# OpenDriveLab/Vista

Measured on NVIDIA H100. Metric: denoised frames/sec at 25x576x1024, 50 EDM steps; UNet step ms, higher is better.
Workload: dtype f16 (fp32 accumulate, fp32 norms/softmax/sampler state)

## Files before the change

vista_b200/csrc/gemm_tc.cu:

```cuda
#include "gemm_tc.cuh"

namespace vb {
extern template const GemmKern* gemm_variants<32>();
extern template const GemmKern* gemm_variants<64>();
extern template const GemmKern* gemm_variants<96>();
extern template const GemmKern* gemm_variants<128>();
extern template const GemmKern* gemm_variants<160>();
extern template const GemmKern* gemm_variants<192>();
extern template const GemmKern* gemm_variants<224>();
extern template const GemmKern* gemm_variants<256>();
}

extern "C" int b200v_gemm(const b200v_gemm_desc* d, void* stream_) {
  using namespace vb;
  cudaStream_t stream = reinterpret_cast<cudaStream_t>(stream_);
  VB_REQUIRE(d && d->a && d->b && d->out, "b200v_gemm: null pointer");
  VB_REQUIRE(d->cin > 0 && d->cin % 64 == 0, "b200v_gemm: cin=%d must be a positive multiple of 64", d->cin);
  VB_REQUIRE(d->ntaps >= 1 && d->ntaps <= 9, "b200v_gemm: ntaps=%d out of range", d->ntaps);
  VB_REQUIRE(d->N > 0 && d->N % 8 == 0, "b200v_gemm: N=%d must be a multiple of 8", d->N);
  VB_REQUIRE(d->tile_n >= 32 && d->tile_n <= 256 && d->tile_n % 32 == 0, "b200v_gemm: tile_n=%d invalid", d->tile_n);
  VB_REQUIRE(d->lda % 8 == 0 && d->ldo % 8 == 0, "b200v_gemm: lda/ldo must be multiples of 8");
  VB_REQUIRE(d->act >= 0 && d->act <= 3, "b200v_gemm: act=%d invalid", d->act);
  VB_REQUIRE(!(d->act == 2 && (d->tile_n % 64 != 0 || d->N % d->tile_n != 0 || d->out_f32)),
             "b200v_gemm: GEGLU needs tile_n %% 64 == 0, N %% tile_n == 0, 16-bit output");
  VB_REQUIRE(!(d->act == 2 && (d->rowvec || d->res1 || d->res2)), "b200v_gemm: GEGLU epilogue takes bias only");
  VB_REQUIRE(!(d->act == 3 && (d->rowvec || d->res1 || d->res2 || d->bf16 || d->out_f32 || d->stats)),
             "b200v_gemm: the GELU epilogue takes bias only, fp16 operands and output (compiled variant)");
  VB_REQUIRE(!d->res1 || d->ld_res1 % 8 == 0, "b200v_gemm: ld_res1 must be a multiple of 8");
  VB_REQUIRE(!d->res2 || d->ld_res2 % 8 == 0, "b200v_gemm: ld_res2 must be a multiple of 8");
  VB_REQUIRE(!d->rowvec || (d->ld_rowvec % 4 == 0 && d->rv_div > 0 && d->rv_mod > 0), "b200v_gemm: bad rowvec args");
  VB_REQUIRE((reinterpret_cast<uintptr_t>(d->a) & 15) == 0 && (reinterpret_cast<uintptr_t>(d->b) & 15) == 0 &&
                 (reinterpret_cast<uintptr_t>(d->out) & 15) == 0,
             "b200v_gemm: a/b/out must be 16-byte aligned");

  TGParams p;
  memset(&p, 0, sizeof(p));
  p.a_mode = d->a_mode;
  p.tokens = d->tokens;
  const long long K = (long long)d->ntaps * d->cin;
  CUtensorMap tmA, tmB;
  if (d->a_mode == 0) {
    VB_REQUIRE(d->ntaps == 1 && d->h_pad == 0, "b200v_gemm: linear mode takes one tap and no halo rows");
    VB_REQUIRE(d->tokens > 0 && d->tokens < (1ll << 31) - 256, "b200v_gemm: tokens out of range");
    p.W = (int)d->tokens; p.H = 1; p.NB = 1;
    p.BW = 128; p.BH = 1; p.BB = 1;
    p.tiles_w = (int)((d->tokens + 127) / 128); p.tiles_h = 1;
    p.m_tiles = p.tiles_w;
    uint64_t dims[2] = {(uint64_t)d->cin, (uint64_t)d->tokens};
    uint64_t strides[1] = {(uint64_t)d->lda * 2};
    uint32_t box[2] = {64, 128};
    uint32_t es[2] = {1, 1};
    if (encode_tmap_16bit(&tmA, d->a, 2, dims, strides, box, es, d->bf16)) return 3;
  } else {
    VB_REQUIRE(d->a_mode == 1 || d->a_mode == 2, "b200v_gemm: a_mode=%d invalid", d->a_mode);
    const long long out_tokens = d->a_mode == 2 ? 4ll * d->tokens : d->tokens;
    VB_REQUIRE(d->W > 0 && d->H > 0 && d->NB > 0 && (long long)d->W * d->H * d->NB == d->tokens &&
                   out_tokens < (1ll << 31) - 256,
               "b200v_gemm: W*H*NB != tokens (or output tokens >= 2^31)");
    VB_REQUIRE(d->a_mode == 1 || (d->h_pad == 0 && d->act == 0 && !d->rowvec && !d->res1 && !d->res2 && !d->bf16 &&
                                  !d->out_f32 && d->s_acc == 1.0f),
               "b200v_gemm: the upsampling mode (a_mode 2) takes bias and fused statistics only, fp16 in and out");
    VB_REQUIRE(d->box_w > 0 && d->box_h > 0 && d->box_b > 0 && d->box_w * d->box_h * d->box_b == 128,
               "b200v_gemm: box_w*box_h*box_b must be 128");
    p.W = d->W; p.H = d->H; p.NB = d->NB;
    p.BW = d->box_w; p.BH = d->box_h; p.BB = d->box_b;
    p.tiles_w = (d->W + p.BW - 1) / p.BW;
    p.tiles_h = (d->H + p.BH - 1) / p.BH;
    const int tiles_b = (d->NB + p.BB - 1) / p.BB;
    p.m_tiles = p.tiles_w * p.tiles_h * tiles_b * (d->a_mode == 2 ? 4 : 1);
    VB_REQUIRE(d->h_pad >= 0 && d->h_pad <= 4, "b200v_gemm: h_pad=%d out of range", d->h_pad);
    const uint64_t He = (uint64_t)d->H + 2ull * d->h_pad;
    uint64_t dims[4] = {(uint64_t)d->cin, (uint64_t)d->W, He, (uint64_t)d->NB};
    uint64_t strides[3] = {(uint64_t)d->lda * 2, (uint64_t)d->lda * 2 * d->W, (uint64_t)d->lda * 2 * d->W * He};
    uint32_t box[4] = {64, (uint32_t)p.BW, (uint32_t)p.BH, (uint32_t)p.BB};
    uint32_t es[4] = {1, 1, 1, 1};
    if (encode_tmap_16bit(&tmA, d->a, 4, dims, strides, box, es, d->bf16)) return 3;
  }
  {
    uint64_t dims[2] = {(uint64_t)K, (uint64_t)d->N};
    uint64_t strides[1] = {(uint64_t)K * 2};
    uint32_t box[2] = {64, (uint32_t)d->tile_n};
    uint32_t es[2] = {1, 1};
    if (encode_tmap_16bit(&tmB, d->b, 2, dims, strides, box, es, d->bf16)) return 3;
  }
  p.ntaps = d->ntaps;
  p.kc_per_tap = d->cin / 64;
  for (int i = 0; i < 9; ++i) {
    p.dh[i] = d->dh[i] + (d->a_mode == 1 ? d->h_pad : 0);
    p.dw[i] = d->dw[i];
  }
  p.N = d->N;
  p.n_tiles = (d->N + d->tile_n - 1) / d->tile_n;
  p.stage_bytes = kABytes + ((d->tile_n * 128 + 1023) / 1024) * 1024;
  constexpr int kMaxSmem = 227 * 1024;
  p.nstages = (kMaxSmem - 2048 - kStagingBytes) / p.stage_bytes;
  if (p.nstages > kMaxStages) p.nstages = kMaxStages;
  const long long kMaxLd = (1ll << 31) - 1;
  VB_REQUIRE(d->ldo * (d->out_f32 ? 4 : 2) <= kMaxLd && d->ld_rowvec * 4 <= kMaxLd && d->ld_res1 * 2 <= kMaxLd &&
                 d->ld_res2 * 2 <= kMaxLd,
             "b200v_gemm: row stride too large");
  for (p.bw_sh = 0; (1 << p.bw_sh) < p.BW; ++p.bw_sh) {}
  for (p.bh_sh = 0; (1 << p.bh_sh) < p.BH; ++p.bh_sh) {}
  p.out = d->out; p.ldo_b = (int)(d->ldo * (d->out_f32 ? 4 : 2)); p.out_f32 = d->out_f32; p.act = d->act;
  p.bias = d->bias;
  p.rowvec = d->rowvec; p.ld_rowvec_b = (int)(d->ld_rowvec * 4); p.rv_div = d->rv_div > 0 ? d->rv_div : 1;
  p.rv_mod = d->rv_mod > 0 ? d->rv_mod : 1;
  p.res1 = d->res1; p.ld_res1_b = (int)(d->ld_res1 * 2); p.s_res1 = d->s_res1;
  p.res2 = d->res2; p.ld_res2_b = (int)(d->ld_res2 * 2); p.s_res2 = d->s_res2;
  p.s_acc = d->s_acc;
  VB_REQUIRE(!(d->res2 && !d->res1), "b200v_gemm: res2 without res1");
  p.stats = d->stats; p.stats_ld = (int)d->stats_ld; p.stats_col0 = d->stats_col0;
  if (d->stats) {
    VB_REQUIRE(!d->bf16 && !d->out_f32 && d->act == 0 && !d->res2 && !(d->rowvec && d->res1),
               "b200v_gemm: fused statistics need fp16 output, act 0, <= 1 residual and no rowvec + residual");
    VB_REQUIRE(d->stats_ld >= d->stats_col0 + d->N && d->stats_col0 % 4 == 0 && d->stats_ld % 4 == 0 &&
                   (reinterpret_cast<uintptr_t>(d->stats) & 15) == 0,
               "b200v_gemm: bad stats_ld / stats_col0 / alignment");
    VB_REQUIRE(d->a_mode == 0 || (p.BB == 1 && d->W % p.BW == 0 && d->H % p.BH == 0 &&
                                  (d->a_mode == 2 || p.BW == d->W || p.BH == 1)),
               "b200v_gemm: fused statistics need token tiles of 128 consecutive tokens, or boxes that tile each frame "
               "in upsampling mode (box %d x %d x %d on %d x %d)",
               p.BW, p.BH, p.BB, d->W, d->H);
  }

  const int smem_bytes = 1024 + 1024 + p.nstages * p.stage_bytes + kStagingBytes;
  int variant = d->bf16 ? 12 : 7;
  if (d->stats) {
    variant = 9 + (d->rowvec ? 2 : (d->res1 ? 1 : 0));
  } else if (!d->bf16 && !d->out_f32) {
    const int nres = (d->res1 ? 1 : 0) + (d->res2 ? 1 : 0);
    if (d->act == 0 && !d->rowvec) variant = nres;
    else if (d->act == 0 && nres <= 1) variant = 3 + nres;
    else if (d->act == 1 && !d->rowvec && nres == 0) variant = 5;
    else if (d->act == 2) variant = 6;
    else if (d->act == 3) variant = 8;
  }
  static const GemmKern* const kByWidth[8] = {gemm_variants<32>(),  gemm_variants<64>(),  gemm_variants<96>(),
                                              gemm_variants<128>(), gemm_variants<160>(), gemm_variants<192>(),
                                              gemm_variants<224>(), gemm_variants<256>()};
  static bool attr_set[64] = {false};
  if (vb::first_use_on_device(attr_set)) {
    for (int w = 0; w < 8; ++w)
      for (int i = 0; i < kGemmVariants; ++i)
        VB_CHECK_CUDA(cudaFuncSetAttribute(kByWidth[w][i], cudaFuncAttributeMaxDynamicSharedMemorySize, kMaxSmem));
  }
  const long long total = (long long)p.m_tiles * p.n_tiles;
  int grid = device_sm_count();
  if (total < grid) grid = (int)total;
  const GemmKern k = kByWidth[d->tile_n / 32 - 1][variant];
  k<<<grid, kGemmThreads, smem_bytes, stream>>>(tmA, tmB, p);
  VB_CHECK_CUDA(cudaGetLastError());
  return 0;
}
```

vista_b200/csrc/gemm_tc.cuh:

```cuda
#pragma once
#include "../../include/vista_b200.h"
#include "host.cuh"
#include "ptx.cuh"

namespace vb {

constexpr int kMaxStages = 8;
constexpr int kABytes = 128 * 64 * 2;
constexpr int kStageBufBytes = 64 * 32 * 4;
constexpr int kStagingBytes = 2 * 2 * kStageBufBytes;
constexpr int kGemmThreads = 384;

struct TGParams {
  int a_mode;
  int W, H, NB;
  int BW, BH, BB;
  int bw_sh, bh_sh;
  int tiles_w, tiles_h;
  int m_tiles, n_tiles;
  int ntaps, kc_per_tap;
  int dh[9], dw[9];
  int N;
  int nstages, stage_bytes;
  long long tokens;
  void* out;
  int ldo_b;
  int out_f32, act;
  const float* bias;
  const float* rowvec;
  int ld_rowvec_b;
  int rv_div, rv_mod;
  const void* res1;
  int ld_res1_b;
  float s_res1;
  const void* res2;
  int ld_res2_b;
  float s_res2;
  float s_acc;
  float* stats;
  int stats_ld, stats_col0;
};

__device__ __forceinline__ float2 unpack2(uint32_t w, int bf16) {
  if (bf16) return make_float2(__uint_as_float(w << 16), __uint_as_float(w & 0xFFFF0000u));
  return __half22float2(*reinterpret_cast<const __half2*>(&w));
}
__device__ __forceinline__ uint32_t pack2(float a, float b, int bf16) {
  if (bf16) {
    __nv_bfloat162 t = __floats2bfloat162_rn(a, b);
    return *reinterpret_cast<uint32_t*>(&t);
  }
  __half2 t = __floats2half2_rn(a, b);
  return *reinterpret_cast<uint32_t*>(&t);
}

template <int TN, bool BF16>
__device__ __forceinline__ void issue_kchunk(float (&acc)[TN / 2], uint64_t adesc, uint64_t bdesc, bool overwrite) {
#pragma unroll
  for (int kk = 0; kk < 4; ++kk)
    wgmma_ss<TN, BF16>(acc, adesc + (uint64_t)(2 * kk), bdesc + (uint64_t)(2 * kk), (overwrite && kk == 0) ? 0 : 1);
}

template <int TN, int ACT_, bool RV_, int NRES_, bool GEN, bool STATS = false, bool BF16 = false>
__global__ void __launch_bounds__(kGemmThreads, 1)
tapgemm_kernel(const __grid_constant__ CUtensorMap tmA, const __grid_constant__ CUtensorMap tmB, const TGParams p) {
  extern __shared__ uint8_t smem_raw[];
  const uint32_t raw = smem_u32(smem_raw);
  uint8_t* smem = smem_raw + (((raw + 1023u) & ~1023u) - raw);
  uint64_t* full = reinterpret_cast<uint64_t*>(smem);
  uint64_t* empty = full + kMaxStages;
  uint8_t* stages = smem + 1024;

  const int warp = threadIdx.x >> 5, lane = threadIdx.x & 31;
  const int KC = p.ntaps * p.kc_per_tap;
  const int total_tiles = p.m_tiles * p.n_tiles;

  if (threadIdx.x == 0) {
    for (int i = 0; i < p.nstages; ++i) {
      mbar_init(&full[i], 1);
      mbar_init(&empty[i], 8);
    }
    fence_barrier_init();
  }
  if (warp == 8 && lane == 0) {
    tma_prefetch_desc(&tmA);
    tma_prefetch_desc(&tmB);
  }
  __syncthreads();

  if (warp >= 8) {
    setmaxnreg_dec<40>();
    if (warp == 8 && lane == 0) {
      int stage = 0;
      uint32_t phase = 0;
      const uint32_t tx = (uint32_t)(kABytes + TN * 128);
      for (int tile = blockIdx.x; tile < total_tiles; tile += gridDim.x) {
        const int m_blk = tile / p.n_tiles, n_blk = tile - m_blk * p.n_tiles;
        const int up = p.a_mode == 2;
        const int box = up ? (m_blk >> 2) : m_blk;
        const int px = up ? (m_blk & 1) : 0, py = up ? ((m_blk >> 1) & 1) : 0;
        const int tw = box % p.tiles_w;
        const int th = (box / p.tiles_w) % p.tiles_h;
        const int tb = box / (p.tiles_w * p.tiles_h);
        const int w0 = tw * p.BW, h0 = th * p.BH, b0 = tb * p.BB;
        const int n0 = n_blk * TN;
        for (int kc = 0; kc < KC; ++kc) {
          mbar_wait_relaxed(&empty[stage], phase ^ 1, 1);
          uint8_t* sA = stages + stage * p.stage_bytes;
          uint8_t* sB = sA + kABytes;
          const int tap = kc / p.kc_per_tap;
          const int c0 = (kc - tap * p.kc_per_tap) * 64;
          mbar_expect_tx(&full[stage], tx);
          const int dw = up ? ((px + p.dw[tap]) >> 1) : p.dw[tap];
          const int dh = up ? ((py + p.dh[tap]) >> 1) : p.dh[tap];
          if (p.a_mode == 0)
            tma_load_2d(sA, &tmA, &full[stage], c0, w0);
          else
            tma_load_4d(sA, &tmA, &full[stage], c0, w0 + dw, h0 + dh, b0);
          tma_load_2d(sB, &tmB, &full[stage], kc * 64, n0);
          if (++stage == p.nstages) {
            stage = 0;
            phase ^= 1;
          }
        }
      }
    }
    return;
  }

  setmaxnreg_inc<232>();
  const int wg = warp >> 2, wq = warp & 3;
  const int act = GEN ? p.act : ACT_;
  const bool has_rv = GEN ? (p.rowvec != nullptr) : RV_;
  const bool has_r1 = GEN ? (p.res1 != nullptr) : (NRES_ >= 1);
  const bool has_r2 = GEN ? (p.res2 != nullptr) : (NRES_ >= 2);
  constexpr bool bf16 = BF16;
  const bool f32o = GEN ? (p.out_f32 != 0) : false;
  const bool has_bias = p.bias != nullptr;
  constexpr int half = TN >> 1;
  const int tile_out_cols = (act == 2) ? half : TN;
  const int n_out_total = (act == 2) ? (p.N >> 1) : p.N;
  const int G = tile_out_cols >> 5;
  const int out_es = f32o ? 4 : 2;
  const char* r1p = reinterpret_cast<const char*>(p.res1);
  const char* r2p = reinterpret_cast<const char*>(p.res2);
  const uint64_t desc0 = make_desc_sw128(smem_u32(stages), 16, 1024);
  const uint32_t stage_step = (uint32_t)p.stage_bytes >> 4;
  const uint32_t stg0 = smem_u32(stages + p.nstages * p.stage_bytes) + wg * 2 * kStageBufBytes;
  const int g = lane >> 2, c = lane & 3;
  const int rh = wq & 1, chh = wq >> 1;
  const int ch = lane & 3, rsub = lane >> 2;
  int stage = 0;
  uint32_t phase = 0;
  uint32_t gcount = 0;

  float acc[TN / 2];
  for (int tile = blockIdx.x; tile < total_tiles; tile += gridDim.x) {
    const int m_blk = tile / p.n_tiles, n_blk = tile - m_blk * p.n_tiles;
    int prev = -1;
    for (int kc = 0; kc < KC; ++kc) {
      mbar_wait(&full[stage], phase, 3);
      const uint64_t ad = desc0 + (uint64_t)(stage * stage_step + wg * 512);
      const uint64_t bd = desc0 + (uint64_t)(stage * stage_step + (kABytes >> 4));
      wgmma_fence();
      issue_kchunk<TN, BF16>(acc, ad, bd, kc == 0);
      wgmma_commit();
      if (prev >= 0) {
        wgmma_wait<1>();
        if (lane == 0) mbar_arrive(&empty[prev]);
      }
      prev = stage;
      if (++stage == p.nstages) {
        stage = 0;
        phase ^= 1;
      }
    }
    wgmma_wait<0>();
    if (lane == 0) mbar_arrive(&empty[prev]);
    fence_regs(acc);

    const int r_own = wg * 64 + rh * 32 + lane;
    int token_own, valid_own;
    if (p.a_mode == 0) {
      token_own = m_blk * 128 + r_own;
      valid_own = token_own < p.tokens;
    } else {
      const int up = p.a_mode == 2;
      const int box = up ? (m_blk >> 2) : m_blk;
      const int tw = box % p.tiles_w;
      const int t2 = box / p.tiles_w;
      const int th = t2 % p.tiles_h;
      const int tb = t2 / p.tiles_h;
      const int ww = r_own & (p.BW - 1), hh = (r_own >> p.bw_sh) & (p.BH - 1), bb = r_own >> (p.bw_sh + p.bh_sh);
      const int w = tw * p.BW + ww, h = th * p.BH + hh, b = tb * p.BB + bb;
      valid_own = (w < p.W) && (h < p.H) && (b < p.NB);
      token_own = up ? ((2 * (b * p.H + h) + ((m_blk >> 1) & 1)) * 2 * p.W + 2 * w + (m_blk & 1))
                     : (b * p.H + h) * p.W + w;
    }
    if (!valid_own) token_own = 0;
    const uint32_t vrows = __ballot_sync(0xffffffffu, valid_own) >> rsub;
    int tok[4], rvrow[4];
    {
      const int rv_own = has_rv ? (token_own / p.rv_div) % p.rv_mod : 0;
#pragma unroll
      for (int i = 0; i < 4; ++i) {
        tok[i] = __shfl_sync(0xffffffffu, token_own, i * 8 + rsub);
        rvrow[i] = has_rv ? __shfl_sync(0xffffffffu, rv_own, i * 8 + rsub) : 0;
      }
    }
    const int n_out_base = n_blk * tile_out_cols;
#pragma unroll
    for (int k = 0; k < TN / 32; ++k) {
      if (k >= G) break;
      const int c0 = k * 32;
      if (n_out_base + c0 >= n_out_total) break;
      const uint32_t stg = stg0 + (gcount & 1) * kStageBufBytes;
      ++gcount;
      float f[16];
#pragma unroll
      for (int j = 0; j < 16; ++j) f[j] = acc[16 * k + j];
      if (act == 2) {
        float gt[16];
        const int kg = (half >> 5) + k;
#pragma unroll
        for (int j = 0; j < 16; ++j) gt[j] = 0.f;
#pragma unroll
        for (int q = 0; q < TN / 32; ++q)
          if (q == kg) {
#pragma unroll
            for (int j = 0; j < 16; ++j) gt[j] = acc[16 * q + j];
          }
        const int nb = n_blk * TN + c0;
#pragma unroll
        for (int ii = 0; ii < 4; ++ii) {
          float2 bv = make_float2(0.f, 0.f), bg = make_float2(0.f, 0.f);
          if (has_bias) {
            bv = __ldg(reinterpret_cast<const float2*>(p.bias + nb + 8 * ii + 2 * c));
            bg = __ldg(reinterpret_cast<const float2*>(p.bias + nb + half + 8 * ii + 2 * c));
          }
          f[4 * ii + 0] = geglu_fast(f[4 * ii + 0] + bv.x, gt[4 * ii + 0] + bg.x);
          f[4 * ii + 1] = geglu_fast(f[4 * ii + 1] + bv.y, gt[4 * ii + 1] + bg.y);
          f[4 * ii + 2] = geglu_fast(f[4 * ii + 2] + bv.x, gt[4 * ii + 2] + bg.x);
          f[4 * ii + 3] = geglu_fast(f[4 * ii + 3] + bv.y, gt[4 * ii + 3] + bg.y);
        }
      }
#pragma unroll
      for (int ii = 0; ii < 4; ++ii) {
        const int chunk = 2 * ii + (c >> 1), sub = (c & 1) * 8;
#pragma unroll
        for (int hr = 0; hr < 2; ++hr) {
          const int row = wq * 16 + g + 8 * hr;
          asm volatile("st.shared.v2.f32 [%0], {%1, %2};" ::"r"(stg + row * 128 + ((chunk ^ (row & 7)) << 4) + sub),
                       "f"(f[4 * ii + 2 * hr]), "f"(f[4 * ii + 2 * hr + 1])
                       : "memory");
        }
      }
      asm volatile("bar.sync %0, 128;" ::"r"(1 + wg) : "memory");
      {
        const int n = n_out_base + c0 + chh * 16 + ch * 4;
        const bool n_ok = n + 4 <= n_out_total;
        float4 bs = make_float4(0.f, 0.f, 0.f, 0.f);
        float sa = 1.0f;
        if (act != 2) {
          sa = p.s_acc;
          if (has_bias && n_ok) {
            const float4 b4 = __ldg(reinterpret_cast<const float4*>(p.bias + n));
            bs = make_float4(b4.x * sa, b4.y * sa, b4.z * sa, b4.w * sa);
          }
        }
        char* obase = reinterpret_cast<char*>(p.out) + (long long)n * out_es;
        const char* r1base = r1p + (long long)n * 2;
        const char* r2base = r2p + (long long)n * 2;
        const char* rvbase = reinterpret_cast<const char*>(p.rowvec) + (long long)n * 4;
        float cs[4] = {0.f, 0.f, 0.f, 0.f}, cq[4] = {0.f, 0.f, 0.f, 0.f};
        float4 v[4], rv[4];
        uint2 u1[4], u2[4];
#pragma unroll
        for (int i = 0; i < 4; ++i) {
          const int row = rh * 32 + i * 8 + rsub;
          const int chunk = chh * 4 + ch;
          asm volatile("ld.shared.v4.f32 {%0, %1, %2, %3}, [%4];"
                       : "=f"(v[i].x), "=f"(v[i].y), "=f"(v[i].z), "=f"(v[i].w)
                       : "r"(stg + row * 128 + ((chunk ^ (row & 7)) << 4)));
          const bool ok = n_ok && ((vrows >> (8 * i)) & 1u);
          rv[i] = make_float4(0.f, 0.f, 0.f, 0.f);
          u1[i] = make_uint2(0, 0);
          u2[i] = make_uint2(0, 0);
          if (has_rv && ok) rv[i] = __ldg(reinterpret_cast<const float4*>(rvbase + (long long)rvrow[i] * p.ld_rowvec_b));
          if (has_r1 && ok) u1[i] = __ldg(reinterpret_cast<const uint2*>(r1base + (long long)tok[i] * p.ld_res1_b));
          if (has_r2 && ok) u2[i] = __ldg(reinterpret_cast<const uint2*>(r2base + (long long)tok[i] * p.ld_res2_b));
        }
#pragma unroll
        for (int i = 0; i < 4; ++i) {
          const bool ok = n_ok && ((vrows >> (8 * i)) & 1u);
          float4 o = v[i];
          if (act != 2) {
            o.x = fmaf(o.x, sa, bs.x); o.y = fmaf(o.y, sa, bs.y); o.z = fmaf(o.z, sa, bs.z); o.w = fmaf(o.w, sa, bs.w);
            if (has_rv) { o.x += rv[i].x; o.y += rv[i].y; o.z += rv[i].z; o.w += rv[i].w; }
            if (act == 1) { o.x = silu_f(o.x); o.y = silu_f(o.y); o.z = silu_f(o.z); o.w = silu_f(o.w); }
            if (!GEN && act == 3) { o.x = gelu_erf_fast(o.x); o.y = gelu_erf_fast(o.y); o.z = gelu_erf_fast(o.z); o.w = gelu_erf_fast(o.w); }
            if (has_r1) {
              const float2 a = unpack2(u1[i].x, bf16), b = unpack2(u1[i].y, bf16);
              o.x = fmaf(p.s_res1, a.x, o.x); o.y = fmaf(p.s_res1, a.y, o.y);
              o.z = fmaf(p.s_res1, b.x, o.z); o.w = fmaf(p.s_res1, b.y, o.w);
            }
            if (has_r2) {
              const float2 a = unpack2(u2[i].x, bf16), b = unpack2(u2[i].y, bf16);
              o.x = fmaf(p.s_res2, a.x, o.x); o.y = fmaf(p.s_res2, a.y, o.y);
              o.z = fmaf(p.s_res2, b.x, o.z); o.w = fmaf(p.s_res2, b.y, o.w);
            }
          }
          if (STATS && ok) {
            cs[0] += o.x; cs[1] += o.y; cs[2] += o.z; cs[3] += o.w;
            cq[0] = fmaf(o.x, o.x, cq[0]); cq[1] = fmaf(o.y, o.y, cq[1]);
            cq[2] = fmaf(o.z, o.z, cq[2]); cq[3] = fmaf(o.w, o.w, cq[3]);
          }
          char* optr = obase + (long long)tok[i] * p.ldo_b;
          if (f32o) {
            if (ok) *reinterpret_cast<float4*>(optr) = o;
          } else {
            const uint2 pk = make_uint2(pack2(o.x, o.y, bf16), pack2(o.z, o.w, bf16));
            if (ok) *reinterpret_cast<uint2*>(optr) = pk;
          }
        }
        if (STATS) {
#pragma unroll
          for (int off = 4; off < 32; off <<= 1) {
#pragma unroll
            for (int q = 0; q < 4; ++q) {
              cs[q] += __shfl_xor_sync(0xffffffffu, cs[q], off);
              cq[q] += __shfl_xor_sync(0xffffffffu, cq[q], off);
            }
          }
          if (rsub == 0 && n_ok) {
            float* dst = p.stats + (((long long)m_blk * 4 + wg * 2 + rh) * p.stats_ld + p.stats_col0 + n) * 2;
            *reinterpret_cast<float4*>(dst) = make_float4(cs[0], cq[0], cs[1], cq[1]);
            *reinterpret_cast<float4*>(dst + 4) = make_float4(cs[2], cq[2], cs[3], cq[3]);
          }
        }
      }
    }
  }
}

using GemmKern = void (*)(const CUtensorMap, const CUtensorMap, const TGParams);
constexpr int kGemmVariants = 13;

template <int TN>
const GemmKern* gemm_variants() {
  static const GemmKern v[kGemmVariants] = {
      tapgemm_kernel<TN, 0, false, 0, false>,       tapgemm_kernel<TN, 0, false, 1, false>,
      tapgemm_kernel<TN, 0, false, 2, false>,       tapgemm_kernel<TN, 0, true, 0, false>,
      tapgemm_kernel<TN, 0, true, 1, false>,        tapgemm_kernel<TN, 1, false, 0, false>,
      tapgemm_kernel<TN, 2, false, 0, false>,       tapgemm_kernel<TN, 0, true, 2, true>,
      tapgemm_kernel<TN, 3, false, 0, false>,       tapgemm_kernel<TN, 0, false, 0, false, true>,
      tapgemm_kernel<TN, 0, false, 1, false, true>, tapgemm_kernel<TN, 0, true, 0, false, true>,
      tapgemm_kernel<TN, 0, true, 2, true, false, true>};
  return v;
}

}
```

vista_b200/csrc/host.cu:

```cuda
#include <stdarg.h>

#include <mutex>

#include "../../include/vista_b200.h"
#include "host.cuh"

namespace vb {

static thread_local char g_err[1024] = "";

void set_error(const char* fmt, ...) {
  va_list ap;
  va_start(ap, fmt);
  vsnprintf(g_err, sizeof(g_err), fmt, ap);
  va_end(ap);
}
const char* last_error() { return g_err; }

int device_sm_count() {
  static int cached[64] = {0};
  int dev = 0;
  if (cudaGetDevice(&dev) != cudaSuccess || dev < 0 || dev >= 64) return 132;
  if (cached[dev] == 0) {
    int n = 0;
    if (cudaDeviceGetAttribute(&n, cudaDevAttrMultiProcessorCount, dev) != cudaSuccess || n <= 0) n = 132;
    cached[dev] = n;
  }
  return cached[dev];
}

typedef CUresult (*EncodeTiledFn)(CUtensorMap*, CUtensorMapDataType, cuuint32_t, void*, const cuuint64_t*,
                                  const cuuint64_t*, const cuuint32_t*, const cuuint32_t*, CUtensorMapInterleave,
                                  CUtensorMapSwizzle, CUtensorMapL2promotion, CUtensorMapFloatOOBfill);

static EncodeTiledFn get_encode_fn() {
  static EncodeTiledFn fn = nullptr;
  static std::once_flag once;
  std::call_once(once, [] {
    void* p = nullptr;
    cudaDriverEntryPointQueryResult q;
    if (cudaGetDriverEntryPoint("cuTensorMapEncodeTiled", &p, cudaEnableDefault, &q) == cudaSuccess &&
        q == cudaDriverEntryPointSuccess)
      fn = reinterpret_cast<EncodeTiledFn>(p);
  });
  return fn;
}

int encode_tmap_16bit(CUtensorMap* out, const void* base, int rank, const uint64_t* dims,
                      const uint64_t* strides_bytes, const uint32_t* box, const uint32_t* elem_strides, int bf16) {
  EncodeTiledFn fn = get_encode_fn();
  if (!fn) {
    set_error("cuTensorMapEncodeTiled entry point not available (driver too old or no GPU)");
    return 1;
  }
  cuuint64_t gdims[5];
  cuuint64_t gstr[4];
  cuuint32_t gbox[5], ges[5];
  for (int i = 0; i < rank; ++i) {
    gdims[i] = dims[i];
    gbox[i] = box[i];
    ges[i] = elem_strides[i];
  }
  for (int i = 0; i + 1 < rank; ++i) gstr[i] = strides_bytes[i];
  CUresult r = fn(out, bf16 ? CU_TENSOR_MAP_DATA_TYPE_BFLOAT16 : CU_TENSOR_MAP_DATA_TYPE_FLOAT16, (cuuint32_t)rank,
                  const_cast<void*>(base), gdims, gstr, gbox, ges, CU_TENSOR_MAP_INTERLEAVE_NONE,
                  CU_TENSOR_MAP_SWIZZLE_128B, CU_TENSOR_MAP_L2_PROMOTION_L2_256B, CU_TENSOR_MAP_FLOAT_OOB_FILL_NONE);
  if (r != CUDA_SUCCESS) {
    set_error("cuTensorMapEncodeTiled failed: CUresult %d (rank %d dims %llu,%llu,%llu,%llu box %u,%u,%u,%u stride0 %llu)",
              (int)r, rank, (unsigned long long)dims[0], (unsigned long long)(rank > 1 ? dims[1] : 0),
              (unsigned long long)(rank > 2 ? dims[2] : 0), (unsigned long long)(rank > 3 ? dims[3] : 0), box[0],
              rank > 1 ? box[1] : 0, rank > 2 ? box[2] : 0, rank > 3 ? box[3] : 0,
              (unsigned long long)(rank > 1 ? strides_bytes[0] : 0));
    return 1;
  }
  return 0;
}

}

extern "C" const char* b200v_last_error(void) { return vb::last_error(); }
extern "C" int b200v_version(void) { return 100; }
extern "C" int b200v_device_info(int32_t* sm_count, int32_t* cc_major, int32_t* cc_minor) {
  int dev = 0;
  VB_CHECK_CUDA(cudaGetDevice(&dev));
  cudaDeviceProp prop;
  VB_CHECK_CUDA(cudaGetDeviceProperties(&prop, dev));
  if (sm_count) *sm_count = prop.multiProcessorCount;
  if (cc_major) *cc_major = prop.major;
  if (cc_minor) *cc_minor = prop.minor;
  return 0;
}
```

vista_b200/csrc/host.cuh:

```cuda
#pragma once
#include <cuda.h>
#include <cuda_runtime.h>
#include <stdint.h>
#include <stdio.h>
#include <string.h>

namespace vb {

void set_error(const char* fmt, ...);
const char* last_error();
int device_sm_count();
inline bool first_use_on_device(bool (&flags)[64]) {
  int dev = 0;
  if (cudaGetDevice(&dev) != cudaSuccess || dev < 0 || dev >= 64) return true;
  if (flags[dev]) return false;
  flags[dev] = true;
  return true;
}

#define VB_CHECK_CUDA(expr)                                                                        \
  do {                                                                                             \
    cudaError_t _e = (expr);                                                                       \
    if (_e != cudaSuccess) {                                                                       \
      vb::set_error("%s:%d CUDA error %d (%s) in %s", __FILE__, __LINE__, (int)_e, cudaGetErrorString(_e), #expr); \
      return 1;                                                                                    \
    }                                                                                              \
  } while (0)

#define VB_REQUIRE(cond, ...)        \
  do {                               \
    if (!(cond)) {                   \
      vb::set_error(__VA_ARGS__);    \
      return 2;                      \
    }                                \
  } while (0)

int encode_tmap_16bit(CUtensorMap* out, const void* base, int rank, const uint64_t* dims,
                      const uint64_t* strides_bytes, const uint32_t* box, const uint32_t* elem_strides, int bf16);

}
```

vista_b200/ops.py:

```python
from __future__ import annotations

import ctypes as C
import os
from typing import Optional, Sequence, Tuple

import torch

from . import lib as _lib

TAPS_3X3 = [(dh, dw) for dh in (-1, 0, 1) for dw in (-1, 0, 1)]
TAPS_T3 = [(-1, 0), (0, 0), (1, 0)]
TAPS_1 = [(0, 0)]


LAUNCHES = 0


def _count(n: int = 1):
    global LAUNCHES
    LAUNCHES += n


TRACE = None

# ... 14 lines not shown
    if PROFILE is not None:
        e0 = torch.cuda.Event(enable_timing=True)
        e1 = torch.cuda.Event(enable_timing=True)
        e0.record()
        _prof_open = (family, detail, flops, nbytes, e0, e1)


def _prof_end():
    global _prof_open
    if PROFILE is not None and _prof_open is not None:
        _prof_open[5].record()
        PROFILE.append(_prof_open)
        _prof_open = None


def profile_summary(records):
    fam, det = {}, {}
    for family, detail, flops, nbytes, e0, e1 in records:
        ms = e0.elapsed_time(e1)
        for table, key in ((fam, family), (det, (family, detail))):
            r = table.setdefault(key, dict(ms=0.0, launches=0, flops=0.0, bytes=0.0))
            r["ms"] += ms
            r["launches"] += 1
            r["flops"] += flops
            r["bytes"] += nbytes
    for table in (fam, det):
        for r in table.values():
            r["tflops"] = r["flops"] / (r["ms"] * 1e-3) / 1e12 if r["ms"] > 0 else 0.0
            r["gbs"] = r["bytes"] / (r["ms"] * 1e-3) / 1e9 if r["ms"] > 0 else 0.0
    return fam, det


def _stream() -> int:
    return torch.cuda.current_stream().cuda_stream


def _ptr(t: Optional[torch.Tensor]) -> Optional[int]:
    return None if t is None else t.data_ptr()


def _rows(t: torch.Tensor) -> Tuple[int, int]:
    assert t.dim() == 2 and t.stride(1) == 1, "token-major 2-D view with unit channel stride expected"
    if t.is_cuda and t.device.index != torch.cuda.current_device():
        raise RuntimeError(f"vista_b200: tensor on cuda:{t.device.index} but the current device is cuda:{torch.cuda.current_device()}; "
                           "wrap the call in torch.cuda.device(tensor.device)")
    return t.shape[0], t.stride(0)


def pick_box(W: int, H: int, NB: int) -> Tuple[int, int, int]:
    best, best_cost = None, None
    for bw in (128, 64, 32, 16, 8, 4, 2, 1):
        for bh in (1, 2, 4, 8, 16, 32, 64, 128):
            if bw * bh > 128:
                continue
            bb = 128 // (bw * bh)
            tiles = -(-W // bw) * -(-H // bh) * -(-NB // bb)
            cost = (tiles, -bw)
            if best_cost is None or cost < best_cost:
                best, best_cost = (bw, bh, bb), cost
    return best


def stats_box(W: int, H: int, NB: int) -> Optional[Tuple[int, int, int]]:
    if W >= 128:
        return (128, 1, 1) if W % 128 == 0 else None
    if 128 % W == 0 and H % (128 // W) == 0:
        return (W, 128 // W, 1)
    return None


def upsample_stats_box(W: int, H: int) -> Optional[Tuple[int, int, int]]:
    for bw in (128, 64, 32, 16, 8, 4, 2, 1):
        if W % bw == 0 and H % (128 // bw) == 0:
            return (bw, 128 // bw, 1)
    return None


def pick_tile_n(N: int, geglu: bool = False) -> int:
    step = 64 if geglu else 32
    best, best_cost = None, None
    for tn in range(256, step - 1, -step):
        if geglu and N % tn:
            continue
        tiles = -(-N // tn)
        cost = (round(tiles * (61.0 + 0.22 * max(tn, 128)), 3), tiles, tiles * tn - N)
        if best_cost is None or cost < best_cost:
            best, best_cost = tn, cost
    if best is None:
        raise ValueError(f"no tile_n for N={N} geglu={geglu}")
    return best


def gemm(a: torch.Tensor, w: torch.Tensor, out: torch.Tensor, *, taps: Sequence[Tuple[int, int]] = TAPS_1,
         geom: Optional[Tuple[int, int, int]] = None, bias: Optional[torch.Tensor] = None,
         rowvec: Optional[torch.Tensor] = None, rv_div: int = 1, rv_mod: int = 1,
         res1: Optional[torch.Tensor] = None, s_res1: float = 1.0,
         res2: Optional[torch.Tensor] = None, s_res2: float = 1.0,
         s_acc: float = 1.0, act: int = 0, tile_n: Optional[int] = None, cin: Optional[int] = None,
         stats: Optional[torch.Tensor] = None, h_pad: int = 0, upsample: bool = False) -> torch.Tensor:
    assert bias is None or bias.dtype == torch.float32, f"gemm: bias must be fp32, got {bias.dtype}"
    assert rowvec is None or rowvec.dtype == torch.float32, f"gemm: rowvec must be fp32, got {rowvec.dtype}"
    for r in (res1, res2):
        assert r is None or r.dtype == a.dtype, f"gemm: residual dtype {r.dtype} != operand dtype {a.dtype}"
    assert act != 2 or s_acc == 1.0, "gemm: the GEGLU epilogue does not scale by s_acc"
    tokens, lda = _rows(a)
    if h_pad:
        assert geom is not None and tokens == geom[2] * (geom[1] + 2 * h_pad) * geom[0]
        tokens = geom[0] * geom[1] * geom[2]
    N, K = w.shape
    ntaps = len(taps)
    cin = cin if cin is not None else K // ntaps
    assert K == ntaps * cin and w.is_contiguous()
    d = _lib.GemmDesc()
    d.a, d.lda, d.tokens = a.data_ptr(), lda, tokens
    out_tokens = 4 * tokens if upsample else tokens
    if geom is None:
        assert ntaps == 1 and not upsample
        d.a_mode = 0
    else:
        d.a_mode = 2 if upsample else 1
        d.W, d.H, d.NB = geom
        assert geom[0] * geom[1] * geom[2] == tokens
        if upsample and stats is not None:
            box = upsample_stats_box(geom[0], geom[1])
            assert box is not None, f"gemm: no box tiles the frames of {geom} for fused statistics"
        else:
            box = pick_box(*geom) if stats is None else stats_box(*geom)
        d.box_w, d.box_h, d.box_b = box
    d.cin, d.ntaps = cin, ntaps
    for i, (dh, dw) in enumerate(taps):
        d.dh[i], d.dw[i] = dh, dw
    d.b, d.N = w.data_ptr(), N
    d.tile_n = tile_n if tile_n is not None else pick_tile_n(N, act == 2)
    d.bf16 = 1 if a.dtype == torch.bfloat16 else 0
    _, ldo = _rows(out)
    d.out, d.ldo, d.out_f32, d.act = out.data_ptr(), ldo, int(out.dtype == torch.float32), act
    d.bias = _ptr(bias)
    if rowvec is not None:
        d.rowvec, d.ld_rowvec, d.rv_div, d.rv_mod = rowvec.data_ptr(), rowvec.stride(0), rv_div, rv_mod
    if res1 is not None:
        d.res1, d.ld_res1, d.s_res1 = res1.data_ptr(), res1.stride(0), s_res1
    if res2 is not None:
        d.res2, d.ld_res2, d.s_res2 = res2.data_ptr(), res2.stride(0), s_res2
    d.s_acc = s_acc
    if stats is not None:
        assert stats.dtype == torch.float32 and stats.dim() == 3 and stats.shape[2] == 2 and stats.stride(2) == 1 \
            and stats.stride(1) == 2 and stats.stride(0) % 2 == 0 and stats.shape[1] >= (N // 2 if act == 2 else N)
        assert stats.shape[0] >= -(-out_tokens // 128) * 4
        d.stats, d.stats_ld, d.stats_col0 = stats.data_ptr(), stats.stride(0) // 2, 0
    assert not upsample or out.shape[0] >= out_tokens
    d.h_pad = h_pad
    _count()
    n_out = N // 2 if act == 2 else N
    _prof_begin("gemm", f"M={out_tokens} N={N} K={K} taps={ntaps} act={act}{' up2x' if upsample else ''}",
                2.0 * out_tokens * N * K,
                2.0 * tokens * cin + 2.0 * N * K + out.element_size() * out_tokens * n_out
                + (2.0 * tokens * n_out if res1 is not None else 0) + (2.0 * tokens * n_out if res2 is not None else 0))
    _lib.check(_lib.load().b200v_gemm(C.byref(d), _stream()), "b200v_gemm")
    _prof_end()
    _trace(f"gemm taps={ntaps} act={act} N={N} K={K}", out)
    return out




def attention_spatial(q, k, v, out, frames: int, seq: int, heads: int, impl: Optional[int] = None):
    l = _lib.load()
    fn = l.b200v_attention_spatial_v3 if impl == 3 else l.b200v_attention_spatial_v7
    _count(1)
    _prof_begin("attn_spatial", f"frames={frames} seq={seq} heads={heads}", 4.0 * 64 * heads * frames * seq * seq,
                2.0 * 4 * frames * seq * heads * 64)
    _lib.check(fn(q.data_ptr(), q.stride(0), k.data_ptr(), k.stride(0), v.data_ptr(), v.stride(0), out.data_ptr(),
                  out.stride(0), frames, seq, heads, _stream()), "b200v_attention_spatial")
    _prof_end()
    _trace("attn_spatial", out)
    return out


def attention_d80(q, k, v, out, batch: int, seq: int, heads: int):
    for t in (q, k, v, out):
        _rows(t)
    _count(1)
    _prof_begin("attn_d80", f"batch={batch} seq={seq} heads={heads}", 4.0 * 80 * heads * batch * seq * seq,
                2.0 * 4 * batch * seq * heads * 80)
    _lib.check(_lib.load().b200v_attention_d80(q.data_ptr(), q.stride(0), k.data_ptr(), k.stride(0), v.data_ptr(),
                                               v.stride(0), out.data_ptr(), out.stride(0), batch, seq, heads, _stream()),
               "b200v_attention_d80")
    _prof_end()
    _trace("attn_d80", out)
    return out


def clip_preprocess(x, out, antialias: bool = True):
    n, c, H, W = x.shape
    assert c == 3 and x.dtype == torch.float32 and x.is_contiguous()
    _, ldo = _rows(out)
    assert out.shape[0] == n * 257 and out.dtype in (torch.float16, torch.float32)
    _count(1)
    _prof_begin("other", f"clip_preprocess n={n} {H}x{W}", 0.0, 4.0 * x.numel() + 2.0 * out.numel())
    _lib.check(_lib.load().b200v_clip_preprocess(x.data_ptr(), n, H, W, int(bool(antialias)), out.data_ptr(), ldo,
                                                 int(out.dtype == torch.float32), _stream()), "b200v_clip_preprocess")
    _prof_end()
    _trace("clip_preprocess", out)
    return out


def attention_temporal(q, k, v, out, nb: int, T: int, S: int, heads: int):
    _count(1)
    _prof_begin("attn_temporal", f"nb={nb} T={T} S={S} heads={heads}", 4.0 * 64 * heads * nb * S * T * T,
                2.0 * 4 * nb * T * S * heads * 64)
    _lib.check(_lib.load().b200v_attention_temporal(q.data_ptr(), q.stride(0), k.data_ptr(), k.stride(0),
                                                    v.data_ptr(), v.stride(0), out.data_ptr(), out.stride(0),
                                                    nb, T, S, heads, _stream()), "b200v_attention_temporal")
    _prof_end()
    _trace("attn_temporal", out)
    return out


def groupnorm_scratch(frames: int, tokens_per_frame: int, groups: int = 32) -> int:
    chunk = _lib.load().b200v_groupnorm_chunk_for(frames, tokens_per_frame)
    return frames * (-(-tokens_per_frame // chunk)) * groups * 2


class GNWorkspace:

    def __init__(self, device, max_stats: int = 4096):
        self.device = device
        self.partials = torch.empty(1 << 16, dtype=torch.float64, device=device)
        self.counters = torch.zeros(max_stats, dtype=torch.int32, device=device)
        self._retired = []

    def reserve(self, n_doubles: int):
        if self.partials.numel() < n_doubles:
            self._retired.append(self.partials)
            self.partials = torch.empty(n_doubles, dtype=torch.float64, device=self.device)


_default_ws = {}


def groupnorm(x, y, frames: int, tokens_per_frame: int, gamma, beta, eps: float, silu: bool,
              stats: Optional[torch.Tensor] = None, frames_per_stat: int = 1, groups: int = 32,
              ws: Optional[GNWorkspace] = None):
    Cc = gamma.numel()
    l = _lib.load()
    if ws is None:
        ws = _default_ws.setdefault(x.device, GNWorkspace(x.device))
    if stats is None:
        stats = torch.empty(frames // frames_per_stat, groups, 2, dtype=torch.float32, device=x.device)
    ws.reserve(groupnorm_scratch(frames, tokens_per_frame, groups))
    assert frames // frames_per_stat <= ws.counters.numel()
    _count(2)
    _prof_begin("groupnorm", f"tokens={frames * tokens_per_frame} C={Cc} fps={frames_per_stat}", 0.0,
                2.0 * 3 * frames * tokens_per_frame * Cc)
    _lib.check(l.b200v_groupnorm_stats(x.data_ptr(), x.stride(0), frames, tokens_per_frame, Cc, groups,
                                       frames_per_stat, eps, ws.partials.data_ptr(), ws.counters.data_ptr(),
                                       stats.data_ptr(), _stream()), "b200v_groupnorm_stats")
    _lib.check(l.b200v_groupnorm_apply(x.data_ptr(), x.stride(0), y.data_ptr(), y.stride(0), frames,
                                       tokens_per_frame, Cc, groups, frames_per_stat, stats.data_ptr(),
                                       gamma.data_ptr(), beta.data_ptr(), int(silu), _stream()),
               "b200v_groupnorm_apply")
    _prof_end()
    _trace(f"groupnorm fps={frames_per_stat}", y)
    return y


def groupnorm_from_partials(partials, frames: int, tokens_per_frame: int, Cc: int, eps: float, stats: Optional[torch.Tensor],
                            frames_per_stat: int = 1, groups: int = 32, raw_sums: Optional[torch.Tensor] = None):
    _count(1)
    _prof_begin("groupnorm", f"from_partials tokens={frames * tokens_per_frame} C={Cc} fps={frames_per_stat}", 0.0,
                4.0 * 2 * (frames * tokens_per_frame // 32) * Cc)
    assert partials.stride(1) == 2 and partials.stride(2) == 1 and partials.shape[1] == Cc
    _lib.check(_lib.load().b200v_groupnorm_from_partials(partials.data_ptr(), partials.stride(0) // 2, frames // frames_per_stat,
                                                         frames_per_stat, tokens_per_frame, Cc, groups, eps, _ptr(stats),
                                                         _ptr(raw_sums), _stream()), "b200v_groupnorm_from_partials")
    _prof_end()
    return stats


def groupnorm_apply(x, y, frames: int, tokens_per_frame: int, gamma, beta, silu: bool, stats: torch.Tensor,
                    frames_per_stat: int = 1, groups: int = 32):
    Cc = gamma.numel()
    _count(1)
    _prof_begin("groupnorm", f"apply tokens={frames * tokens_per_frame} C={Cc} fps={frames_per_stat}", 0.0,
                2.0 * 2 * frames * tokens_per_frame * Cc)
    _lib.check(_lib.load().b200v_groupnorm_apply(x.data_ptr(), x.stride(0), y.data_ptr(), y.stride(0), frames,
                                                 tokens_per_frame, Cc, groups, frames_per_stat, stats.data_ptr(),
                                                 gamma.data_ptr(), beta.data_ptr(), int(silu), _stream()),
               "b200v_groupnorm_apply")
    _prof_end()
    _trace(f"groupnorm(apply) fps={frames_per_stat}", y)
    return y


def groupnorm_sums(x, frames: int, tokens_per_frame: int, Cc: int, sums: torch.Tensor, frames_per_stat: int,
                   groups: int = 32, ws: Optional[GNWorkspace] = None):
    l = _lib.load()
    if ws is None:
        ws = _default_ws.setdefault(x.device, GNWorkspace(x.device))
    ws.reserve(groupnorm_scratch(frames, tokens_per_frame, groups))
    _count(1)
    _prof_begin("groupnorm", f"sums tokens={frames * tokens_per_frame} C={Cc} fps={frames_per_stat}", 0.0,
                2.0 * frames * tokens_per_frame * Cc)
    _lib.check(l.b200v_groupnorm_sums(x.data_ptr(), x.stride(0), frames, tokens_per_frame, Cc, groups, frames_per_stat,
                                      ws.partials.data_ptr(), ws.counters.data_ptr(), sums.data_ptr(), _stream()),
               "b200v_groupnorm_sums")
    _prof_end()
# ... 304 lines not shown
```

Baseline: 1.302.

## Prefetch GEMM epilogue residuals via TMA into shared-memory ring with dedicated producer warp

Adds TMA tensor maps for the residual inputs, plus a dedicated producer warp that streams 128x32 residual boxes into a ring of shared-memory slots ahead of the epilogue. The epilogue then reads residuals from shared memory instead of doing scattered __ldg global loads, so residual fetch latency overlaps with the MMA mainloop. In exchange, residual slots take shared memory away from the operand pipeline and may drop one stage. It also adds mbarrier handshakes, and the unswizzled smem reads may hit bank conflicts.

```diff
diff --git a/vista_b200/csrc/gemm_tc.cu b/vista_b200/csrc/gemm_tc.cu
--- a/vista_b200/csrc/gemm_tc.cu
+++ b/vista_b200/csrc/gemm_tc.cu
@@ -30,15 +30,18 @@
   VB_REQUIRE(!d->res2 || d->ld_res2 % 8 == 0, "b200v_gemm: ld_res2 must be a multiple of 8");
   VB_REQUIRE(!d->rowvec || (d->ld_rowvec % 4 == 0 && d->rv_div > 0 && d->rv_mod > 0), "b200v_gemm: bad rowvec args");
   VB_REQUIRE((reinterpret_cast<uintptr_t>(d->a) & 15) == 0 && (reinterpret_cast<uintptr_t>(d->b) & 15) == 0 &&
-                 (reinterpret_cast<uintptr_t>(d->out) & 15) == 0,
-             "b200v_gemm: a/b/out must be 16-byte aligned");
+                 (reinterpret_cast<uintptr_t>(d->out) & 15) == 0 && (reinterpret_cast<uintptr_t>(d->res1) & 15) == 0 &&
+                 (reinterpret_cast<uintptr_t>(d->res2) & 15) == 0,
+             "b200v_gemm: a/b/out/res1/res2 must be 16-byte aligned");
 
   TGParams p;
   memset(&p, 0, sizeof(p));
   p.a_mode = d->a_mode;
   p.tokens = d->tokens;
   const long long K = (long long)d->ntaps * d->cin;
-  CUtensorMap tmA, tmB;
+  CUtensorMap tmA, tmB, tmR1, tmR2;
+  memset(&tmR1, 0, sizeof(tmR1));
+  memset(&tmR2, 0, sizeof(tmR2));
   if (d->a_mode == 0) {
     VB_REQUIRE(d->ntaps == 1 && d->h_pad == 0, "b200v_gemm: linear mode takes one tap and no halo rows");
     VB_REQUIRE(d->tokens > 0 && d->tokens < (1ll << 31) - 256, "b200v_gemm: tokens out of range");
@@ -93,8 +96,17 @@
   p.n_tiles = (d->N + d->tile_n - 1) / d->tile_n;
   p.stage_bytes = kABytes + ((d->tile_n * 128 + 1023) / 1024) * 1024;
   constexpr int kMaxSmem = 227 * 1024;
-  p.nstages = (kMaxSmem - 2048 - kStagingBytes) / p.stage_bytes;
+  const int budget = kMaxSmem - 2048 - kStagingBytes;
+  p.nstages = budget / p.stage_bytes;
   if (p.nstages > kMaxStages) p.nstages = kMaxStages;
+  const int nres = (d->res1 ? 1 : 0) + (d->res2 ? 1 : 0);
+  const int rslot_bytes = nres * kResBoxBytes;
+  p.rslots = 0;
+  if (nres) {
+    if (budget - p.nstages * p.stage_bytes < 2 * rslot_bytes) --p.nstages;
+    p.rslots = (budget - p.nstages * p.stage_bytes) / rslot_bytes;
+    if (p.rslots > kMaxResSlots) p.rslots = kMaxResSlots;
+  }
   const long long kMaxLd = (1ll << 31) - 1;
   VB_REQUIRE(d->ldo * (d->out_f32 ? 4 : 2) <= kMaxLd && d->ld_rowvec * 4 <= kMaxLd && d->ld_res1 * 2 <= kMaxLd &&
                  d->ld_res2 * 2 <= kMaxLd,
@@ -105,10 +117,27 @@
   p.bias = d->bias;
   p.rowvec = d->rowvec; p.ld_rowvec_b = (int)(d->ld_rowvec * 4); p.rv_div = d->rv_div > 0 ? d->rv_div : 1;
   p.rv_mod = d->rv_mod > 0 ? d->rv_mod : 1;
-  p.res1 = d->res1; p.ld_res1_b = (int)(d->ld_res1 * 2); p.s_res1 = d->s_res1;
-  p.res2 = d->res2; p.ld_res2_b = (int)(d->ld_res2 * 2); p.s_res2 = d->s_res2;
+  p.res1 = d->res1; p.s_res1 = d->s_res1;
+  p.res2 = d->res2; p.s_res2 = d->s_res2;
   p.s_acc = d->s_acc;
   VB_REQUIRE(!(d->res2 && !d->res1), "b200v_gemm: res2 without res1");
+  for (int r = 0; r < nres; ++r) {
+    const void* base = r == 0 ? d->res1 : d->res2;
+    const uint64_t ldb = (uint64_t)(r == 0 ? d->ld_res1 : d->ld_res2) * 2;
+    CUtensorMap* tm = r == 0 ? &tmR1 : &tmR2;
+    uint32_t es[4] = {1, 1, 1, 1};
+    if (d->a_mode == 0) {
+      uint64_t dims[2] = {(uint64_t)d->N, (uint64_t)d->tokens};
+      uint64_t strides[1] = {ldb};
+      uint32_t box[2] = {32, 128};
+      if (encode_tmap_16bit(tm, base, 2, dims, strides, box, es, d->bf16, 0)) return 3;
+    } else {
+      uint64_t dims[4] = {(uint64_t)d->N, (uint64_t)d->W, (uint64_t)d->H, (uint64_t)d->NB};
+      uint64_t strides[3] = {ldb, ldb * d->W, ldb * d->W * d->H};
+      uint32_t box[4] = {32, (uint32_t)p.BW, (uint32_t)p.BH, (uint32_t)p.BB};
+      if (encode_tmap_16bit(tm, base, 4, dims, strides, box, es, d->bf16, 0)) return 3;
+    }
+  }
   p.stats = d->stats; p.stats_ld = (int)d->stats_ld; p.stats_col0 = d->stats_col0;
   if (d->stats) {
     VB_REQUIRE(!d->bf16 && !d->out_f32 && d->act == 0 && !d->res2 && !(d->rowvec && d->res1),
@@ -123,7 +152,7 @@
                p.BW, p.BH, p.BB, d->W, d->H);
   }
 
-  const int smem_bytes = 1024 + 1024 + p.nstages * p.stage_bytes + kStagingBytes;
+  const int smem_bytes = 1024 + 1024 + p.nstages * p.stage_bytes + kStagingBytes + p.rslots * rslot_bytes;
   int variant = d->bf16 ? 12 : 7;
   if (d->stats) {
     variant = 9 + (d->rowvec ? 2 : (d->res1 ? 1 : 0));
@@ -148,7 +177,7 @@
   int grid = device_sm_count();
   if (total < grid) grid = (int)total;
   const GemmKern k = kByWidth[d->tile_n / 32 - 1][variant];
-  k<<<grid, kGemmThreads, smem_bytes, stream>>>(tmA, tmB, p);
+  k<<<grid, kGemmThreads, smem_bytes, stream>>>(tmA, tmB, tmR1, tmR2, p);
   VB_CHECK_CUDA(cudaGetLastError());
   return 0;
 }
diff --git a/vista_b200/csrc/gemm_tc.cuh b/vista_b200/csrc/gemm_tc.cuh
--- a/vista_b200/csrc/gemm_tc.cuh
+++ b/vista_b200/csrc/gemm_tc.cuh
@@ -6,7 +6,9 @@
 namespace vb {
 
 constexpr int kMaxStages = 8;
+constexpr int kMaxResSlots = 4;
 constexpr int kABytes = 128 * 64 * 2;
+constexpr int kResBoxBytes = 128 * 32 * 2;
 constexpr int kStageBufBytes = 64 * 32 * 4;
 constexpr int kStagingBytes = 2 * 2 * kStageBufBytes;
 constexpr int kGemmThreads = 384;
@@ -22,6 +24,7 @@
   int dh[9], dw[9];
   int N;
   int nstages, stage_bytes;
+  int rslots;
   long long tokens;
   void* out;
   int ldo_b;
@@ -31,10 +34,8 @@
   int ld_rowvec_b;
   int rv_div, rv_mod;
   const void* res1;
-  int ld_res1_b;
   float s_res1;
   const void* res2;
-  int ld_res2_b;
   float s_res2;
   float s_acc;
   float* stats;
@@ -63,13 +64,20 @@
 
 template <int TN, int ACT_, bool RV_, int NRES_, bool GEN, bool STATS = false, bool BF16 = false>
 __global__ void __launch_bounds__(kGemmThreads, 1)
-tapgemm_kernel(const __grid_constant__ CUtensorMap tmA, const __grid_constant__ CUtensorMap tmB, const TGParams p) {
+tapgemm_kernel(const __grid_constant__ CUtensorMap tmA, const __grid_constant__ CUtensorMap tmB,
+               const __grid_constant__ CUtensorMap tmR1, const __grid_constant__ CUtensorMap tmR2, const TGParams p) {
   extern __shared__ uint8_t smem_raw[];
   const uint32_t raw = smem_u32(smem_raw);
   uint8_t* smem = smem_raw + (((raw + 1023u) & ~1023u) - raw);
   uint64_t* full = reinterpret_cast<uint64_t*>(smem);
   uint64_t* empty = full + kMaxStages;
+  uint64_t* rfull = empty + kMaxStages;
+  uint64_t* rempty = rfull + kMaxResSlots;
   uint8_t* stages = smem + 1024;
+  uint8_t* rbuf = stages + p.nstages * p.stage_bytes + kStagingBytes;
+  const bool has_r1 = GEN ? (p.res1 != nullptr) : (NRES_ >= 1);
+  const bool has_r2 = GEN ? (p.res2 != nullptr) : (NRES_ >= 2);
+  const int rslot_bytes = has_r2 ? 2 * kResBoxBytes : kResBoxBytes;
 
   const int warp = threadIdx.x >> 5, lane = threadIdx.x & 31;
   const int KC = p.ntaps * p.kc_per_tap;
@@ -80,11 +88,19 @@
       mbar_init(&full[i], 1);
       mbar_init(&empty[i], 8);
     }
+    for (int i = 0; i < p.rslots; ++i) {
+      mbar_init(&rfull[i], 1);
+      mbar_init(&rempty[i], 8);
+    }
     fence_barrier_init();
   }
   if (warp == 8 && lane == 0) {
     tma_prefetch_desc(&tmA);
     tma_prefetch_desc(&tmB);
+  }
+  if (warp == 9 && lane == 0 && has_r1) {
+    tma_prefetch_desc(&tmR1);
+    if (has_r2) tma_prefetch_desc(&tmR2);
   }
   __syncthreads();
 
@@ -124,6 +140,31 @@
           }
         }
       }
+    } else if (warp == 9 && lane == 0 && has_r1) {
+      int slot = 0;
+      uint32_t phase = 0;
+      for (int tile = blockIdx.x; tile < total_tiles; tile += gridDim.x) {
+        const int m_blk = tile / p.n_tiles, n_blk = tile - m_blk * p.n_tiles;
+        const int tw = m_blk % p.tiles_w;
+        const int th = (m_blk / p.tiles_w) % p.tiles_h;
+        const int tb = m_blk / (p.tiles_w * p.tiles_h);
+        for (int n = n_blk * TN; n < n_blk * TN + TN && n < p.N; n += 32) {
+          mbar_wait_relaxed(&rempty[slot], phase ^ 1, 4);
+          uint8_t* dst = rbuf + slot * rslot_bytes;
+          mbar_expect_tx(&rfull[slot], (uint32_t)rslot_bytes);
+          if (p.a_mode == 0) {
+            tma_load_2d(dst, &tmR1, &rfull[slot], n, m_blk * 128);
+            if (has_r2) tma_load_2d(dst + kResBoxBytes, &tmR2, &rfull[slot], n, m_blk * 128);
+          } else {
+            tma_load_4d(dst, &tmR1, &rfull[slot], n, tw * p.BW, th * p.BH, tb * p.BB);
+            if (has_r2) tma_load_4d(dst + kResBoxBytes, &tmR2, &rfull[slot], n, tw * p.BW, th * p.BH, tb * p.BB);
+          }
+          if (++slot == p.rslots) {
+            slot = 0;
+            phase ^= 1;
+          }
+        }
+      }
     }
     return;
   }
@@ -132,8 +173,6 @@
   const int wg = warp >> 2, wq = warp & 3;
   const int act = GEN ? p.act : ACT_;
   const bool has_rv = GEN ? (p.rowvec != nullptr) : RV_;
-  const bool has_r1 = GEN ? (p.res1 != nullptr) : (NRES_ >= 1);
-  const bool has_r2 = GEN ? (p.res2 != nullptr) : (NRES_ >= 2);
   constexpr bool bf16 = BF16;
   const bool f32o = GEN ? (p.out_f32 != 0) : false;
   const bool has_bias = p.bias != nullptr;
@@ -142,8 +181,6 @@
   const int n_out_total = (act == 2) ? (p.N >> 1) : p.N;
   const int G = tile_out_cols >> 5;
   const int out_es = f32o ? 4 : 2;
-  const char* r1p = reinterpret_cast<const char*>(p.res1);
-  const char* r2p = reinterpret_cast<const char*>(p.res2);
   const uint64_t desc0 = make_desc_sw128(smem_u32(stages), 16, 1024);
   const uint32_t stage_step = (uint32_t)p.stage_bytes >> 4;
   const uint32_t stg0 = smem_u32(stages + p.nstages * p.stage_bytes) + wg * 2 * kStageBufBytes;
@@ -153,6 +190,9 @@
   int stage = 0;
   uint32_t phase = 0;
   uint32_t gcount = 0;
+  int rslot = 0;
+  uint32_t rphase = 0;
+  const uint32_t rbuf0 = smem_u32(rbuf);
 
   float acc[TN / 2];
   for (int tile = blockIdx.x; tile < total_tiles; tile += gridDim.x) {
@@ -256,6 +296,7 @@
         }
       }
       asm volatile("bar.sync %0, 128;" ::"r"(1 + wg) : "memory");
+      if (has_r1) mbar_wait(&rfull[rslot], rphase, 5);
       {
         const int n = n_out_base + c0 + chh * 16 + ch * 4;
         const bool n_ok = n + 4 <= n_out_total;
@@ -269,8 +310,7 @@
           }
         }
         char* obase = reinterpret_cast<char*>(p.out) + (long long)n * out_es;
-        const char* r1base = r1p + (long long)n * 2;
-        const char* r2base = r2p + (long long)n * 2;
+        const uint32_t rbase = rbuf0 + rslot * rslot_bytes + (wg * 64 + rh * 32 + rsub) * 64 + (chh * 16 + ch * 4) * 2;
         const char* rvbase = reinterpret_cast<const char*>(p.rowvec) + (long long)n * 4;
         float cs[4] = {0.f, 0.f, 0.f, 0.f}, cq[4] = {0.f, 0.f, 0.f, 0.f};
         float4 v[4], rv[4];
@@ -287,8 +327,11 @@
           u1[i] = make_uint2(0, 0);
           u2[i] = make_uint2(0, 0);
           if (has_rv && ok) rv[i] = __ldg(reinterpret_cast<const float4*>(rvbase + (long long)rvrow[i] * p.ld_rowvec_b));
-          if (has_r1 && ok) u1[i] = __ldg(reinterpret_cast<const uint2*>(r1base + (long long)tok[i] * p.ld_res1_b));
-          if (has_r2 && ok) u2[i] = __ldg(reinterpret_cast<const uint2*>(r2base + (long long)tok[i] * p.ld_res2_b));
+          if (has_r1)
+            asm volatile("ld.shared.v2.b32 {%0, %1}, [%2];" : "=r"(u1[i].x), "=r"(u1[i].y) : "r"(rbase + i * 512));
+          if (has_r2)
+            asm volatile("ld.shared.v2.b32 {%0, %1}, [%2];"
+                         : "=r"(u2[i].x), "=r"(u2[i].y) : "r"(rbase + kResBoxBytes + i * 512));
         }
 #pragma unroll
         for (int i = 0; i < 4; ++i) {
@@ -338,12 +381,21 @@
             *reinterpret_cast<float4*>(dst + 4) = make_float4(cs[2], cq[2], cs[3], cq[3]);
           }
         }
-      }
-    }
-  }
-}
-
-using GemmKern = void (*)(const CUtensorMap, const CUtensorMap, const TGParams);
+        if (has_r1) {
+          fence_proxy_async_smem();
+          __syncwarp();
+          if (lane == 0) mbar_arrive(&rempty[rslot]);
+          if (++rslot == p.rslots) {
+            rslot = 0;
+            rphase ^= 1;
+          }
+        }
+      }
+    }
+  }
+}
+
+using GemmKern = void (*)(const CUtensorMap, const CUtensorMap, const CUtensorMap, const CUtensorMap, const TGParams);
 constexpr int kGemmVariants = 13;
 
 template <int TN>
diff --git a/vista_b200/csrc/host.cu b/vista_b200/csrc/host.cu
--- a/vista_b200/csrc/host.cu
+++ b/vista_b200/csrc/host.cu
@@ -47,7 +47,8 @@
 }
 
 int encode_tmap_16bit(CUtensorMap* out, const void* base, int rank, const uint64_t* dims,
-                      const uint64_t* strides_bytes, const uint32_t* box, const uint32_t* elem_strides, int bf16) {
+                      const uint64_t* strides_bytes, const uint32_t* box, const uint32_t* elem_strides, int bf16,
+                      int swizzle128) {
   EncodeTiledFn fn = get_encode_fn();
   if (!fn) {
     set_error("cuTensorMapEncodeTiled entry point not available (driver too old or no GPU)");
@@ -64,7 +65,8 @@
   for (int i = 0; i + 1 < rank; ++i) gstr[i] = strides_bytes[i];
   CUresult r = fn(out, bf16 ? CU_TENSOR_MAP_DATA_TYPE_BFLOAT16 : CU_TENSOR_MAP_DATA_TYPE_FLOAT16, (cuuint32_t)rank,
                   const_cast<void*>(base), gdims, gstr, gbox, ges, CU_TENSOR_MAP_INTERLEAVE_NONE,
-                  CU_TENSOR_MAP_SWIZZLE_128B, CU_TENSOR_MAP_L2_PROMOTION_L2_256B, CU_TENSOR_MAP_FLOAT_OOB_FILL_NONE);
+                  swizzle128 ? CU_TENSOR_MAP_SWIZZLE_128B : CU_TENSOR_MAP_SWIZZLE_NONE, CU_TENSOR_MAP_L2_PROMOTION_L2_256B,
+                  CU_TENSOR_MAP_FLOAT_OOB_FILL_NONE);
   if (r != CUDA_SUCCESS) {
     set_error("cuTensorMapEncodeTiled failed: CUresult %d (rank %d dims %llu,%llu,%llu,%llu box %u,%u,%u,%u stride0 %llu)",
               (int)r, rank, (unsigned long long)dims[0], (unsigned long long)(rank > 1 ? dims[1] : 0),
diff --git a/vista_b200/csrc/host.cuh b/vista_b200/csrc/host.cuh
--- a/vista_b200/csrc/host.cuh
+++ b/vista_b200/csrc/host.cuh
@@ -36,6 +36,7 @@
   } while (0)
 
 int encode_tmap_16bit(CUtensorMap* out, const void* base, int rank, const uint64_t* dims,
-                      const uint64_t* strides_bytes, const uint32_t* box, const uint32_t* elem_strides, int bf16);
+                      const uint64_t* strides_bytes, const uint32_t* box, const uint32_t* elem_strides, int bf16,
+                      int swizzle128 = 1);
 
 }
diff --git a/vista_b200/ops.py b/vista_b200/ops.py
--- a/vista_b200/ops.py
+++ b/vista_b200/ops.py
@@ -190,7 +190,8 @@
     d.h_pad = h_pad
     _count()
     n_out = N // 2 if act == 2 else N
-    _prof_begin("gemm", f"M={out_tokens} N={N} K={K} taps={ntaps} act={act}{' up2x' if upsample else ''}",
+    _prof_begin("gemm", f"M={out_tokens} N={N} K={K} taps={ntaps} act={act} res={(res1 is not None) + (res2 is not None)}"
+                f"{' up2x' if upsample else ''}",
                 2.0 * out_tokens * N * K,
                 2.0 * tokens * cin + 2.0 * N * K + out.element_size() * out_tokens * n_out
                 + (2.0 * tokens * n_out if res1 is not None else 0) + (2.0 * tokens * n_out if res2 is not None else 0))
```

After: 1.337, median of 6. +2.7%, better.
